# kscalelabs/gym-kmanip

Hardware: AMD Instinct MI355X
Metric: env steps/sec (whole node), KManipSoloArm @4096 envs, 1/2/4/8 MI355X (higher is better)
Workload: dtype f64

## Files before the change

gym_kmanip_amd/csrc/kmanip_api.hip:

```cpp
#include <hip/hip_runtime.h>

#include <cstdio>
#include <cstdlib>
#include <cmath>
#include <cstring>
#include <new>
#include <string>
#include <vector>

#include "kmanip_device.hpp"

#define KM_VERSION "kmanip-hip 0.33 (gfx950, f64)"

static thread_local std::string g_create_error;

struct KHandle_ {
  KModelDesc desc;
  KDeviceModel* dmodel = nullptr;
  KDeviceState st{};
  int device = 0;
  int num_envs = 0;
  std::string err;
  std::vector<hipEvent_t> ev;
  std::vector<char> ev_render;
  bool timing = false;
  int timing_every = 1;
  long timing_count = 0;
  double* rd_rec[2] = {nullptr, nullptr};
  int rd_sel = 0;
  int timed_steps = 0;
  double* qpos_snap[2] = {nullptr, nullptr};
  int render_src = -1;
  bool last_step_timed = false;
  int step_cam = -1, step_h = 0, step_w = 0;
  float* step_depth = nullptr;
// ... 1006 lines not shown
```

gym_kmanip_amd/csrc/kmanip_dyn_env.hpp:

```cpp
#pragma once
template <int NL, int G, int SOLVER>
__device__ __forceinline__ void step1_products(Ws<NL>& w, const LModel<NL>& lm, const KModelDesc* m, int sub,
                                               CReg<NL>& cr, real invm, Prof& pf) {
  real kin[15];
  fk_parallel<NL, G>(w, lm, sub, G == 16 ? kin : nullptr);
  pf.ph(0);
  real FN[6];
  const int split = G == 32 ? lm.split : 0;
  int bli = -1, bbase = 0;
  if constexpr (G == 32) {
    const int row = (threadIdx.x >> 4) & 1, c = threadIdx.x & 15;
    bbase = row ? split : 0;
    bli = (split && c < (row ? NL - split : split)) ? bbase + c : -1;
    if (split) {
      for (int e = sub; e < (int)(sizeof(w.Minv) / sizeof(real)); e += G) (&w.Minv[0][0])[e] = 0.0;
    }
  }
  if constexpr (G == 16) bias_bodies_rows<NL, NL>(w, lm, m, sub < NL ? sub : -1, 0, sub == NL, FN, kin);
  else if (split) {
    bias_bodies_rows<NL, KM_BLOCK_MAX>(w, lm, m, bli, bbase, false, FN);
    if (sub == NL) cube_bias<NL>(w, m);
  }
  else bias_bodies_parallel<NL, G>(w, lm, m, sub);
  pf.ph(1);
// ... 42 lines not shown
  real v = 0;
  if (sub < NV) {
    v = v0 + dt * a;
    w.qvel[sub] = v;
    w.warm[sub] = a;
    if (sub < NL + 3) w.qpos[sub] = qp + dt * v;
  }
  real ax[3] = {gbcast<G, NL + 3>(v), gbcast<G, NL + 4>(v), gbcast<G, NL + 5>(v)};
  if (sub == 0) {
    real ang = dt * normalize3_fast(ax), qr[4], qn[4];
    axis_angle2quat(qr, ax, ang);
    normalize4_fast(q);
    qmul(qn, q, qr);
    normalize4_fast(qn);
    w.qpos[NL + 3] = qn[0]; w.qpos[NL + 4] = qn[1]; w.qpos[NL + 5] = qn[2]; w.qpos[NL + 6] = qn[3];
  }
  GSYNC();
}

__device__ __forceinline__ real clip1(real x) { return fmin(fmax(x, -1.0), 1.0); }

template <int NL, int G>
__device__ __forceinline__ void write_obs(const Ws<NL>& w, const LModel<NL>& lm, const KModelDesc* m, int sub, double* obs_row) {
  for (int i = sub; i < NL; i += G) {
    obs_row[i] = clip1((w.qpos[i] - lm.range[i][0]) / (lm.range[i][1] - lm.range[i][0]));
    obs_row[NL + i] = clip1(w.qvel[i] / m->max_q_vel);
  }
  for (int c = sub; c < 7; c += G) {
    if (c < 3) obs_row[2 * NL + c] = clip1((w.qpos[NL + c] - m->cube_spawn_lo[c]) / (m->cube_spawn_hi[c] - m->cube_spawn_lo[c]));
    else obs_row[2 * NL + c] = w.qpos[NL + c];
  }
}

__device__ __forceinline__ real lerp_unfused(real lo, real hi, real u) {
#pragma clang fp contract(off)
  const real d = hi - lo;
  const real p = d * u;
  return lo + p;
}

#if KM_VAR_PAR
__device__ __forceinline__ real ep_inertia(const KModelDesc* m, real mass, int k) {
#pragma clang fp contract(off)
  return m->cube_inertia[k] * (mass / m->cube_mass);
}
__device__ __forceinline__ void ep_mass_consts(const KDeviceModel* dm, real mass, const real (&I)[3], int nv, real& cw1, real& mi) {
#pragma clang fp contract(off)
  cw1 = ((1.0 / I[0] + 1.0 / I[1]) + 1.0 / I[2]) / 3.0;
  mi = mass == dm->d.cube_mass ? dm->d.meaninertia : ((dm->trace_robot + 3.0 * mass) + ((I[0] + I[1]) + I[2])) / nv;
}
template <int NL>
__device__ __forceinline__ real ep_invm(const KModelDesc* m, const real (&p)[KM_EP_N], int sub) {
  if (sub < NL || sub >= Dim<NL>::NV) return 0;
// ... 95 lines not shown
#pragma unroll
  for (int k = 0; k < KL; k++) { const int i = sub + G * k; c[k] = st.ctrl[(size_t)(i < NL ? i : NL - 1) * NE + env]; }
#pragma unroll
  for (int k = 0; k < KQ; k++) { const int i = sub + G * k; if (i < NQ) { w.qpos[i] = q[k]; if (i < NL) w.qpos_ik[i] = q[k]; } }
#pragma unroll
  for (int k = 0; k < KV; k++) { const int i = sub + G * k; if (i < NV) { w.qvel[i] = v[k]; w.warm[i] = wm[k]; } }
#pragma unroll
  for (int k = 0; k < KL; k++) { const int i = sub + G * k; if (i < NL) w.ctrl[i] = (real)(float)c[k]; }
  if (sub == 0) { w.bad = 0; w.work = 0; }
}
template <int NL> struct LdsIO {
  Ws<NL>& w; const KDeviceState& st; int env;
  __device__ __forceinline__ real qpos(int i) const { return w.qpos[i]; }
  __device__ __forceinline__ void set_ctrl(int i, real v) { w.ctrl[i] = v; }
  __device__ __forceinline__ void set_qpos_ik(int i, real v) { w.qpos_ik[i] = v; }
  __device__ __forceinline__ void set_diag(int arm, int nfev, int status) {
    st.ik_nfev[(size_t)arm * st.num_envs + env] = nfev; st.ik_status[(size_t)arm * st.num_envs + env] = status;
  }
};
template <int NL, int G>
__device__ __forceinline__ void store_state(const Ws<NL>& w, const KDeviceState& st, int env, int sub) {
  constexpr int NV = Dim<NL>::NV, NQ = Dim<NL>::NQ;
  const int NE = st.num_envs;
  for (int i = sub; i < NQ; i += G) st.qpos[(size_t)i * NE + env] = w.qpos[i];
  for (int i = sub; i < NV; i += G) { st.qvel[(size_t)i * NE + env] = w.qvel[i]; st.warm[(size_t)i * NE + env] = w.warm[i]; }
  for (int i = sub; i < NL; i += G) st.ctrl[(size_t)i * NE + env] = w.ctrl[i];
}

template <int NL>
__device__ __forceinline__ void stage_model(LModel<NL>& lm, const KDeviceModel* dm) {
  static_assert(sizeof(LModel<NL>) % 16 == 0 && sizeof(LModel<NL>) <= KM_LMODEL_MAX, "the staged image is copied in 16-byte pieces");
  constexpr int N16 = (int)(sizeof(LModel<NL>) / 16);
  const uint4* src = reinterpret_cast<const uint4*>(dm->staged);
  uint4* dst = reinterpret_cast<uint4*>(&lm);
  uint4 v[(N16 + 63) / 64];
#pragma unroll
  for (int k = 0; k < (N16 + 63) / 64; k++) { const int i = threadIdx.x + 64 * k; v[k] = src[i < N16 ? i : N16 - 1]; }
#pragma unroll
  for (int k = 0; k < (N16 + 63) / 64; k++) { const int i = threadIdx.x + 64 * k; if (i < N16) dst[i] = v[k]; }
  __syncthreads();
}
template <int NL>
__device__ __forceinline__ void build_lmodel(LModel<NL>& lm, const KDeviceModel* dm) {
  const KModelDesc* m = &dm->d;
  for (int i = threadIdx.x; i < NL; i += 64) {
    lm.parent[i] = m->link_parent[i]; lm.jtype[i] = m->jnt_type[i]; lm.forcelimited[i] = m->forcelimited[i];
    lm.anc[i] = dm->x.anc_mask[i]; lm.desc[i] = dm->x.desc_mask[i];
    for (int k = 0; k < 4; k++) lm.jump[k][i] = dm->x.jump[k][i];
    if (i == 0) {
// ... 14 lines not shown
        lm.sphA[0][sp] = (cw + lw) + muc * muc * (cw + lw);
        lm.sphA[1][sp] = lw + mud * mud * lw;
      }
    }
    if (i < Dim<NL>::NSPH) {
      const int sp = i < m->nsphere ? i : 0;
      lm.sph_link[i] = m->sphere_link[sp]; lm.sph_rad[i] = m->sphere_radius[sp];
      for (int c = 0; c < 3; c++) { lm.sph_pos[i][c] = m->sphere_pos[sp][c]; lm.sph_seg[i][c] = m->sphere_seg[sp][c]; }
      if (i == 0) lm.nsph = m->nsphere < Dim<NL>::NSPH ? m->nsphere : Dim<NL>::NSPH;
    }
    lm.dofw[i] = m->dof_invweight0[i];
    lm.floss[i] = m->frictionloss[i]; lm.kp[i] = m->kp[i]; lm.mass[i] = m->mass[i]; lm.q_home[i] = m->q_home[i];
    for (int c = 0; c < 3; c++) { lm.pos[i][c] = m->link_pos[i][c]; lm.jaxis[i][c] = m->jnt_axis[i][c]; lm.com[i][c] = m->com[i][c]; lm.inertia[i][c] = m->inertia[i][c]; }
    for (int c = 0; c < 4; c++) lm.quat[i][c] = m->link_quat[i][c];
    { real qn[4] = {m->link_quat[i][0], m->link_quat[i][1], m->link_quat[i][2], m->link_quat[i][3]}, Rm[9]; normalize4(qn); quat2mat(Rm, qn); for (int c = 0; c < 9; c++) lm.R[i][c] = Rm[c]; }
    for (int c = 0; c < 2; c++) { lm.range[i][c] = m->jnt_range[i][c]; lm.ctrlrange[i][c] = m->ctrlrange[i][c]; lm.forcerange[i][c] = m->forcerange[i][c]; }
  }
  __syncthreads();
}

template <int NL, int G>
__device__ __forceinline__ real env_reward(Ws<NL>& w, const KModelDesc* m, int sub) {
  constexpr int NV = Dim<NL>::NV;
  real v2 = gsum<G>(sub < NV ? w.qvel[sub] * w.qvel[sub] : 0.0);
  GSYNC();
  real rew = -m->reward_vel_penalty * km_sqrt(v2);
  for (int arm = 1; arm >= 0; arm--) {
    if (!m->arm_present[arm] || !m->arm_has_grip[arm]) continue;
    const int l = m->arm_site_link[arm];
    real so[3] = {m->arm_site_pos[arm][0], m->arm_site_pos[arm][1], m->arm_site_pos[arm][2]}, sp[3];
    mat_vec3(sp, w.k.xmat[l], so);
    real df[3] = {w.qpos[NL] - (sp[0] + w.k.xpos[l][0]), w.qpos[NL + 1] - (sp[1] + w.k.xpos[l][1]), w.qpos[NL + 2] - (sp[2] + w.k.xpos[l][2])};
    rew += m->reward_grip_dist * (1.0 / (km_sqrt(dot3(df, df)) + m->epsilon));
  }
  if (m->touch_reward_enabled && (w.contact_mask & KM_CON_FINGERS_CUBE(NL))) {
    rew += m->reward_touch_cube;
    if (!w.touch_ct) rew += m->reward_lift_cube;
  }
  return rew;
}
```

gym_kmanip_amd/csrc/kmanip_dyn_newton.hpp:

```cpp
#pragma once

enum { KM_SUB_ALL = 0, KM_SUB_ARM = 1, KM_SUB_CUBE = 2 };
template <int NL, int S> struct SubSet {
  static constexpr int D0 = S == KM_SUB_CUBE ? NL : 0, D1 = S == KM_SUB_ARM ? NL : NL + 6;
  static constexpr int kind(int c) { return slot_kind<NL>(c); }
  static constexpr bool slot(int c) { return S == KM_SUB_ALL || (S == KM_SUB_ARM ? kind(c) == 2 : kind(c) == 0); }
  static constexpr int c0(int c) { const int k = kind(c); const int lo = k == 0 ? NL : 0; return lo > D0 ? lo : D0; }
  static constexpr int c1(int c) { const int k = kind(c); const int hi = k == 2 ? NL : NL + 6; return hi < D1 ? hi : D1; }
};

template <int G, int N, int D0, int D1>
__device__ __forceinline__ void chol_rows(real (&h)[N], real& invd, int sub, int& bad) {
  static_for<D0, D1>([&](auto kc) {
    constexpr int k = decltype(kc)::value;
    real dk = gbcast<G, k>(h[k]);
    if (!(dk > 0)) { bad = 1; dk = 1; }
    const real inv = rsqrt_nr(dk);
    const real lik = h[k] * inv;
    h[k] = lik;
    if (sub == k) invd = inv;
    const BSrc<G> lsrc = bsrc<G>(lik);
    fnmac_cols<G, k + 1, D1>(h, lsrc, lik);
    if constexpr (k + 2 >= D1 && k + 1 < D1) dpp_settle(h[k + 1]);
  });
// ... 330 lines not shown
template <int NL, int G, int S>
__device__ __forceinline__ void slot_grad(const CReg<NL>& cr, uint32_t act, const real (&F)[4], real& grad) {
  constexpr int NC = Dim<NL>::NC;
  static_assert(NC <= 16, "the slot lanes sit in the group's first DPP row");
  using SS = SubSet<NL, S>;
  const real F0 = row0<G>(F[0]), F1 = row0<G>(F[1]), F2 = row0<G>(F[2]), F3 = row0<G>(F[3]);
  static_for<0, NC>([&](auto cc) {
    constexpr int c = decltype(cc)::value;
    if constexpr (SS::slot(c)) {
      if ((act >> c) & 1u) {
        real g2 = 0;
        if constexpr (slot_kind<NL>(c) == 2) dppfma_acc3<c>(g2, F0, cr.jb[c][0], F1, cr.jb[c][1], F2, cr.jb[c][2]);
        else dppfma_acc4<c>(g2, F0, cr.jb[c][0], F1, cr.jb[c][1], F2, cr.jb[c][2], F3, cr.jb[c][3]);
        grad -= g2;
      }
    }
  });
}
template <int NL, int S> __device__ __forceinline__ bool slot_lane_in(int sub) {
  constexpr int NC = Dim<NL>::NC, NSS = Dim<NL>::NSS;
  return S == KM_SUB_ALL ? sub < NC : (S == KM_SUB_ARM ? (sub >= 4 + NSS && sub < NC) : sub < 4);
}

template <int NL, int G, bool CS>
__device__ __forceinline__ void newton_eval_sl(const Ws<NL>& w, int sub, const CReg<NL>& cr, real a, real a_s, real Mr, real& grad, int& qf,
                                               int& ql, real (&u)[4], real (&W)[7], real& c0, real& c1, real& cs) {
  constexpr int NV = Dim<NL>::NV;
  const uint32_t act = w.cact;
  const SlotC& sc = cr.sc;
  slot_project<NL, G, KM_SUB_ALL>(w, cr, act, sub, a, u);
#pragma unroll
  for (int k = 0; k < 4; k++) u[k] -= sc.A[k];
  real F[4];
  const real cslot = slot_eval<true>(sc, u, F, W);
  real csl = 0;
  if constexpr (CS) {
    real us[4], Fs[4], Ws_[7];
    slot_project<NL, G, KM_SUB_ALL>(w, cr, act, sub, a_s, us);
#pragma unroll
    for (int k = 0; k < 4; k++) us[k] -= sc.A[k];
    csl = slot_eval<false>(sc, us, Fs, Ws_);
  }
  grad = Mr;
  qf = 0; ql = 0;
  {
    real co = 0.5 * (a - a_s) * Mr;
    if (cr.fl > 0) { real f; co += row_eval(0, a - cr.areff, cr.Rf, cr.Df, cr.fl, f, qf); grad -= f; }
    if (cr.sg != 0) { real f; co += row_eval(1, cr.sg * a - cr.arefl, cr.Rl, cr.Dl, 0.0, f, ql); grad -= cr.sg * f; }
    c0 = sub < NL ? co : 0.0; c1 = (sub >= NL && sub < NV) ? co : 0.0;
    if constexpr (CS) {
      real f; int qd;
      if (cr.fl > 0) csl += row_eval(0, a_s - cr.areff, cr.Rf, cr.Df, cr.fl, f, qd);
      if (cr.sg != 0) csl += row_eval(1, cr.sg * a_s - cr.arefl, cr.Rl, cr.Dl, 0.0, f, qd);
    }
  }
  c1 += sub < 4 ? cslot : 0.0; c0 += sub < 4 ? 0.0 : cslot;
  slot_grad<NL, G, KM_SUB_ALL>(cr, act, F, grad);
  cs = csl;
}

// ... 294 lines not shown
    if constexpr (JOINT) { if (prob == KM_SUB_ALL) { pf.cnt(lone_it ? 44 : 45, 1); pf.it_end(lone_it ? 46 : 47); } }
#endif
    if (improvement < tol || gradient < tol || w.bad || iter + 1 >= maxit) {
      if (!(JOINT && prob == KM_SUB_ARM)) break;
      enter(KM_SUB_CUBE); cost = cost_b;
      if (small()) break;
      iter = -1;
    }
  }
}

template <int NL, int G>
__device__ __forceinline__ real solve_newton_sl(Ws<NL>& w, const LModel<NL>& lm, const KModelDesc* m, int sub, CReg<NL>& cr, real a_s,
                                                real invm, Prof& pf) {
  constexpr int NV = Dim<NL>::NV;
  const uint32_t act = w.cact;
  const real warm = sub < NV ? w.warm[sub] : 0.0;
  const real mdiag = (sub >= NL && sub < NV) ? 1.0 / invm : 0.0;
  real grad; int qf, ql;
  real u[4], W[7];
  real c0, c1, csl;
  real a = warm;
  real Mr = mass_mul<NL, G>(cr, sub, mdiag, warm - a_s);
  newton_eval_sl<NL, G, true>(w, sub, cr, a, a_s, Mr, grad, qf, ql, u, W, c0, c1, csl);
  real c3[3] = {csl, c0, c1};
  gsum_n<G, 3>(c3);
  const real cs = c3[0];
  real cost0 = c3[1], cost1 = c3[2];
  pf.ph(8);
  if (!(cost0 + cost1 < cs)) {
    a = a_s; Mr = 0;
    real dummy;
    newton_eval_sl<NL, G, false>(w, sub, cr, a, a_s, Mr, grad, qf, ql, u, W, c0, c1, dummy);
    real c2[2] = {c0, c1};
    gsum_n<G, 2>(c2);
    cost0 = c2[0]; cost1 = c2[1];
    pf.ph(38);
  }
  constexpr uint32_t FC_MASK = ((1u << Dim<NL>::NSS) - 1u) << 4;
  const bool coupled = (act & FC_MASK) != 0;
  if constexpr (G == 16) {
    int resume = KM_SUB_ARM, riter = 0;
    real rcost = cost0;
    if (__any(coupled)) {
      resume = 0;
      newton_loop_sl<NL, G, KM_SUB_ALL, true>(w, lm, m, sub, cr, mdiag, a_s, a, Mr, coupled ? cost0 + cost1 : cost0, grad, qf, ql, u, W, pf, !coupled, cost1,
                                              0, &resume, &rcost, &riter);
    }
    if (resume == KM_SUB_ARM) newton_loop_sl<NL, G, KM_SUB_ARM>(w, lm, m, sub, cr, mdiag, a_s, a, Mr, rcost, grad, qf, ql, u, W, pf, false, 0, riter);
    if (resume != 0) newton_loop_sl<NL, G, KM_SUB_CUBE>(w, lm, m, sub, cr, mdiag, a_s, a, Mr, resume == KM_SUB_ARM ? cost1 : rcost, grad, qf, ql, u, W, pf,
                                                        false, 0, resume == KM_SUB_ARM ? 0 : riter);
  } else {
    if (!coupled) newton_loop_sl<NL, G, KM_SUB_ARM>(w, lm, m, sub, cr, mdiag, a_s, a, Mr, cost0, grad, qf, ql, u, W, pf);
    if (coupled) newton_loop_sl<NL, G, KM_SUB_ALL>(w, lm, m, sub, cr, mdiag, a_s, a, Mr, cost0 + cost1, grad, qf, ql, u, W, pf);
    else newton_loop_sl<NL, G, KM_SUB_CUBE>(w, lm, m, sub, cr, mdiag, a_s, a, Mr, cost1, grad, qf, ql, u, W, pf);
  }
// ... 38 lines not shown
```

gym_kmanip_amd/csrc/kmanip_ik_coop.hip:

```cpp
#include "kmanip_ik_coop.hpp"

template <int N>
__global__ __launch_bounds__(64) void k_ik_coop_standalone(const KDeviceModel* __restrict__ dm, int arm, int n, int nq,
                                                           double* qpos, const double* goal_pos, const double* goal_quat,
                                                           double* q_out, int32_t* nfev_o, int32_t* status_o) {
  const KModelDesc* m = &dm->d;
  const int slot = threadIdx.x / GS, c = threadIdx.x % GS;
  const int e = blockIdx.x * PPW + slot;
  if (c >= GI || e >= n) return;
  double* qp = qpos + (size_t)e * nq;
  CoopCtx<N> P;
  Prof pf;
  P.m = m; P.ax = &dm->x; P.arm = arm; P.c = c; P.on = c < N; P.pf = &pf;
  coop_chain_setup<N>(P);
  const int q = m->arm_q_id[arm][P.on ? c : 0];
  const real x0 = P.on ? qp[q] : 0.0;
  P.q_prev = x0; P.q_home = m->q_home[q]; P.lb = m->jnt_range[q][0]; P.ub = m->jnt_range[q][1];
  P.qfix = (P.clen > N) ? qp[dm->x.chain_link[arm][P.clen - 1]] : 0.0;
  for (int k = 0; k < 3; k++) P.goal_pos[k] = goal_pos[3 * e + k];
  for (int k = 0; k < 4; k++) P.goal_quat[k] = goal_quat[4 * e + k];
  real xl;
  int nfev, status;
  const real qo = coop_ik_solve<N>(P, x0, xl, &nfev, &status);
  KM_GSYNC();
// ... 11 lines not shown
  else
    hipLaunchKernelGGL(k_ik_coop_standalone<6>, grid, dim3(64), 0, stream, dm, arm, n, nq, qpos, goal_pos, goal_quat, q_out, nfev, status);
}

template <int N>
__global__ __launch_bounds__(64) void k_ik_eval_coop(const KDeviceModel* __restrict__ dm, int arm, int n, int nq, const double* qpos,
                                                     const double* goal_pos, const double* goal_quat, double* res, double* jac) {
  const KModelDesc* m = &dm->d;
  const int slot = threadIdx.x / GS, c = threadIdx.x % GS;
  const int e = blockIdx.x * PPW + slot;
  if (c >= GI || e >= n) return;
  const double* qp = qpos + (size_t)e * nq;
  CoopCtx<N> P;
  Prof pf;
  P.m = m; P.ax = &dm->x; P.arm = arm; P.c = c; P.on = c < N; P.pf = &pf;
  coop_chain_setup<N>(P);
  const int q = m->arm_q_id[arm][P.on ? c : 0];
  const real x0 = P.on ? qp[q] : 0.0;
  P.q_prev = x0; P.q_home = m->q_home[q]; P.lb = m->jnt_range[q][0]; P.ub = m->jnt_range[q][1];
  P.qfix = (P.clen > N) ? qp[dm->x.chain_link[arm][P.clen - 1]] : 0.0;
  for (int k = 0; k < 3; k++) P.goal_pos[k] = goal_pos[3 * e + k];
  for (int k = 0; k < 4; k++) P.goal_quat[k] = goal_quat[4 * e + k];
  real ft[6], Jc[6];
  coop_eval<N, true>(P, x0, ft, Jc, nullptr, nullptr);
  constexpr int M = 6 + 2 * N;
  double* r = res + (size_t)e * M;
  double* J = jac + (size_t)e * M * N;
  if (c == 0) for (int k = 0; k < 6; k++) r[k] = ft[k];
  if (P.on) {
    r[6 + c] = m->ik_res_reg_prev * (x0 - P.q_prev);
    r[6 + N + c] = m->ik_res_reg_home * (x0 - P.q_home);
    for (int k = 0; k < M; k++) J[k * N + c] = 0;
    for (int k = 0; k < 6; k++) J[k * N + c] = Jc[k];
    J[(6 + c) * N + c] = m->ik_jac_reg;
    J[(6 + N + c) * N + c] = m->ik_jac_reg;
  }
}

void kmanip_launch_ik_eval_coop(const KDeviceModel* dm, const KModelDesc& hd, int arm, int n, const double* qpos,
                                const double* goal_pos, const double* goal_quat, double* res, double* jac, hipStream_t stream) {
  int nq = hd.nlink + 7;
  dim3 grid((n + PPW - 1) / PPW);
  if (hd.arm_nq[arm] == 7) hipLaunchKernelGGL(k_ik_eval_coop<7>, grid, dim3(64), 0, stream, dm, arm, n, nq, qpos, goal_pos, goal_quat, res, jac);
  else hipLaunchKernelGGL(k_ik_eval_coop<6>, grid, dim3(64), 0, stream, dm, arm, n, nq, qpos, goal_pos, goal_quat, res, jac);
}
```

gym_kmanip_amd/csrc/kmanip_ik_coop.hpp:

```cpp
#pragma once
#include "kmanip_device.hpp"

#define GI 8
#define GS 16
#define PPW (64 / GS)

__device__ __forceinline__ real gsum8(real v) {
#pragma clang fp contract(off)
  v += dpp_f64<0x141>(v);
  v += dpp_f64<0xB1>(v);
  v += dpp_f64<0x4E>(v);
  return v;
}
template <int N> __device__ __forceinline__ void gsum8_n(real (&v)[N]) {
#pragma clang fp contract(off)
  real t[N];
#pragma unroll
  for (int i = 0; i < N; i++) t[i] = dpp_f64<0x141>(v[i]);
#pragma unroll
  for (int i = 0; i < N; i++) v[i] += t[i];
#pragma unroll
  for (int i = 0; i < N; i++) t[i] = dpp_f64<0xB1>(v[i]);
#pragma unroll
  for (int i = 0; i < N; i++) v[i] += t[i];
// ... 24 lines not shown
  const KModelDesc* m;
  const KModelAux* ax;
  int arm, c;
  bool on;
  real goal_pos[3], goal_quat[4];
  real qfix;
  real q_prev, q_home, lb, ub;
  real cR[9], cp[3];
  int clen, cslide;
  Prof* pf;
};
template <int N>
__device__ __forceinline__ void coop_chain_setup(CoopCtx<N>& P) {
  P.clen = P.ax->chain_len[P.arm];
  const int k = P.c < P.clen ? P.c : 0;
  const int l = P.ax->chain_link[P.arm][k];
#pragma unroll
  for (int i = 0; i < 9; i++) P.cR[i] = P.ax->chain_R[P.arm][k][i];
  P.cp[0] = P.m->link_pos[l][0]; P.cp[1] = P.m->link_pos[l][1]; P.cp[2] = P.m->link_pos[l][2];
  P.cslide = P.m->jnt_type[l] == KM_JNT_SLIDE;
}
template <int S> __device__ __forceinline__ real shr8(real v) { return dpp_f64<0x110 + S>(v); }

template <int N, bool JAC>
__device__ __forceinline__ void coop_eval(const CoopCtx<N>& P, real x, real* ft, real* Jc, real* sp_out, real* smat_out) {
  const KModelDesc* m = P.m;
  const int arm = P.arm;
  const int clen = P.clen;
  real R[9], p[3];
  {
    const real q = P.on ? x : P.qfix;
    p[0] = P.cp[0]; p[1] = P.cp[1]; p[2] = P.cp[2];
    if (P.c >= clen) {
      R[0] = 1; R[1] = 0; R[2] = 0; R[3] = 0; R[4] = 1; R[5] = 0; R[6] = 0; R[7] = 0; R[8] = 1;
      p[0] = 0; p[1] = 0; p[2] = 0;
    } else if (P.cslide) {
#pragma unroll
      for (int i = 0; i < 9; i++) R[i] = P.cR[i];
      p[0] += R[2] * q; p[1] += R[5] * q; p[2] += R[8] * q;
    } else {
      real sn, cs;
      km_sincos(q, &sn, &cs);
#pragma unroll
      for (int i = 0; i < 3; i++) {
        R[3 * i] = cs * P.cR[3 * i] + sn * P.cR[3 * i + 1];
        R[3 * i + 1] = cs * P.cR[3 * i + 1] - sn * P.cR[3 * i];
        R[3 * i + 2] = P.cR[3 * i + 2];
      }
// ... 1 lines not shown
  }
  static_for<0, 3>([&](auto rc) {
    constexpr int S = 1 << decltype(rc)::value;
    real A[9], pa[3];
#pragma unroll
    for (int i = 0; i < 9; i++) A[i] = shr8<S>(R[i]);
    pa[0] = shr8<S>(p[0]); pa[1] = shr8<S>(p[1]); pa[2] = shr8<S>(p[2]);
    if (P.c >= S) {
      real t[3], Rn[9];
      mat_vec3(t, A, p);
      p[0] = t[0] + pa[0]; p[1] = t[1] + pa[1]; p[2] = t[2] + pa[2];
#pragma unroll
      for (int i = 0; i < 3; i++)
#pragma unroll
        for (int j = 0; j < 3; j++) Rn[3 * i + j] = A[3 * i] * R[j] + A[3 * i + 1] * R[3 + j] + A[3 * i + 2] * R[6 + j];
#pragma unroll
      for (int i = 0; i < 9; i++) R[i] = Rn[i];
    }
  });
  real mat[9], pos[3];
#pragma unroll
  for (int i = 0; i < 9; i++) mat[i] = bcast8<GI - 1>(R[i]);
  pos[0] = bcast8<GI - 1>(p[0]); pos[1] = bcast8<GI - 1>(p[1]); pos[2] = bcast8<GI - 1>(p[2]);
  const real anc[3] = {p[0], p[1], p[2]}, axw[3] = {R[2], R[5], R[8]};
  real sp[3], smat[9], cur[4], rq[3];
  real so[3] = {m->arm_site_pos[arm][0], m->arm_site_pos[arm][1], m->arm_site_pos[arm][2]};
  const double* Rs = P.ax->site_R[arm];
  mat_vec3(sp, mat, so);
  sp[0] += pos[0]; sp[1] += pos[1]; sp[2] += pos[2];
#pragma unroll
  for (int i = 0; i < 3; i++)
#pragma unroll
    for (int j = 0; j < 3; j++) smat[3 * i + j] = mat[3 * i] * Rs[j] + mat[3 * i + 1] * Rs[3 + j] + mat[3 * i + 2] * Rs[6 + j];
  mat2quat(cur, smat);
  real sn_h, ac_h;
  sub_quat_sc(rq, P.goal_quat, cur, sn_h, ac_h);
  if (sp_out) { sp_out[0] = sp[0]; sp_out[1] = sp[1]; sp_out[2] = sp[2]; }
  if (smat_out) {
#pragma unroll
    for (int i = 0; i < 9; i++) smat_out[i] = smat[i];
  }
  ft[0] = sp[0] - P.goal_pos[0]; ft[1] = sp[1] - P.goal_pos[1]; ft[2] = sp[2] - P.goal_pos[2];
  ft[3] = rq[0] * m->ik_res_rad; ft[4] = rq[1] * m->ik_res_rad; ft[5] = rq[2] * m->ik_res_rad;
  if (JAC) {
    real axs[3] = {rq[0], rq[1], rq[2]};
    real half = 0.5 * normalize3_fast(axs);
    real coef = 1.0 - (half < 6e-8 ? 1.0 : half * ac_h / sn_h);
    if (!P.on) { Jc[0] = 0; Jc[1] = 0; Jc[2] = 0; Jc[3] = 0; Jc[4] = 0; Jc[5] = 0; }
    else if (P.cslide) { Jc[0] = axw[0]; Jc[1] = axw[1]; Jc[2] = axw[2]; Jc[3] = 0; Jc[4] = 0; Jc[5] = 0; }
    else {
      real r[3] = {sp[0] - anc[0], sp[1] - anc[1], sp[2] - anc[2]}, jp[3];
      cross3(jp, axw, r);
      Jc[0] = jp[0]; Jc[1] = jp[1]; Jc[2] = jp[2];
      real uu[3], cx[3];
      matT_vec3(uu, smat, axw);
      cross3(cx, axs, uu);
      const real du = dot3(axs, uu);
#pragma unroll
      for (int i = 0; i < 3; i++) Jc[3 + i] = -m->ik_jac_rad * ((uu[i] + half * cx[i]) + coef * (axs[i] * du - uu[i]));
    }
  }
}

template <int N>
__device__ __forceinline__ real coop_cost(const CoopCtx<N>& P, real x, const real* ft) {
  real a = P.m->ik_res_reg_prev * (x - P.q_prev), b = P.m->ik_res_reg_home * (x - P.q_home);
  real loc = P.on ? a * a + b * b : 0.0;
  real s = gsum8(loc);
#pragma unroll
  for (int r = 0; r < 6; r++) s += ft[r] * ft[r];
  return 0.5 * s;
}
template <int N>
__device__ __forceinline__ real coop_grad(const CoopCtx<N>& P, real x, const real* ft, const real* Jc) {
  if (!P.on) return 0.0;
  real s = 0;
#pragma unroll
  for (int r = 0; r < 6; r++) s += Jc[r] * ft[r];
  return s + P.m->ik_jac_reg * (P.m->ik_res_reg_prev * (x - P.q_prev) + P.m->ik_res_reg_home * (x - P.q_home));
}

template <int N> struct TrFac { real h[N], ut[N], invd; };
template <int N>
__device__ __forceinline__ bool chol_coop(const real (&arow)[N], const real (&e)[N], real alpha, int c, TrFac<N>& F) {
// ... 77 lines not shown
template <int N>
__device__ __forceinline__ real ldl_fwd(const TrFacB<N>& F, real b) {
  static_for<0, N / 2>([&](auto kc) {
    constexpr int p = 2 * decltype(kc)::value, q = p + 1;
    if constexpr (q + 1 < N) { const real zb = b; dppfma_row2n<p, q>(b, zb, F.h[p], F.h[q]); }
  });
  return b;
}
template <int N>
__device__ __forceinline__ real ldl_mid(const TrFacB<N>& F, real z) {
  const real zp = dpp_f64<0xB1>(z);
  return __builtin_fma(F.dd, z, F.dx * zp);
}
template <int N>
__device__ __forceinline__ real ldl_bwd(const TrFacB<N>& F, real x) {
  if constexpr (N & 1) { const real xb = x; dppfma1<true, N - 1>(x, xb, F.ut[N - 1]); }
  static_for<0, N / 2>([&](auto kc) {
    constexpr int k = N / 2 - 1 - decltype(kc)::value, p = 2 * k, q = p + 1;
    if constexpr (k > 0) { const real xb = x; dppfma_row2n<p, q>(x, xb, F.ut[p], F.ut[q]); }
  });
  return x;
}

template <int N>
__device__ __forceinline__ void solve_tr_coop(const real (&arow)[N], const real (&e)[N], int c, real g_h, real Delta, real& alpha, real& p) {
  const real ng = -g_h;
#ifdef KM_IK_CHOLESKY
  TrFac<N> F;
  auto factor = [&](real al) { return chol_coop<N>(arow, e, al, c, F); };
  auto solve = [&](real rhs) { return tr_bwd<N>(F, tr_fwd<N>(F, rhs)); };
  auto ainv_norm2 = [&](real v) { const real q = tr_fwd<N>(F, v); return gsum8(q * q); };
#else
  TrFacB<N> F;
  auto factor = [&](real al) { return ldl_coop<N>(arow, e, al, c, F); };
  auto solve = [&](real rhs) { return ldl_bwd<N>(F, ldl_mid<N>(F, ldl_fwd<N>(F, rhs))); };
  auto ainv_norm2 = [&](real v) { const real z = ldl_fwd<N>(F, v); return gsum8(z * ldl_mid<N>(F, z)); };
#endif
  const bool full_rank = factor(0.0);
  real pn = 0;
  if (full_rank) {
    p = solve(ng);
    pn = km_sqrt(gsum8(p * p));
    if (pn <= Delta) { alpha = 0.0; return; }
  }
  const real iDelta = frcp(Delta);
  real alpha_upper = km_sqrt(gsum8(g_h * g_h)) * iDelta, alpha_lower = 0.0;
  if (full_rank) {
    const real phi = pn - Delta, phip = -ainv_norm2(p) * frcp(pn);
    alpha_lower = -phi * frcp(phip);
  }
  if (!full_rank && alpha == 0) alpha = fmax(0.001 * alpha_upper, sqrt(alpha_lower * alpha_upper));
  for (int it = 0; it < 10; it++) {
    if (alpha < alpha_lower || alpha > alpha_upper) alpha = fmax(0.001 * alpha_upper, sqrt(alpha_lower * alpha_upper));
    factor(alpha);
    p = solve(ng);
    pn = km_sqrt(gsum8(p * p));
    const real phi = pn - Delta, phip = -ainv_norm2(p) * frcp(pn);
    if (phi < 0) alpha_upper = alpha;
    const real ratio = phi * frcp(phip);
    alpha_lower = fmax(alpha_lower, alpha - ratio);
    alpha -= (phi + Delta) * ratio * iDelta;
    if (fabs(phi) < 0.01 * Delta) break;
  }
  factor(alpha);
  p = solve(ng);
  p *= Delta * rsqrt_nr(gsum8(p * p));
}

__device__ __forceinline__ void min_quad_1d_c(real a, real b, real lo, real hi, real c, real& t_out, real& y_out) {
  real tb = lo, yb = lo * (a * lo + b) + c;
  real y1 = hi * (a * hi + b) + c;
// ... 80 lines not shown
  agh *= ag_stride;
  if (p_value < r_value && p_value < ag_value) { step_h = pht; return -p_value; }
  if (r_value < p_value && r_value < ag_value) { step_h = rh; return -r_value; }
  step_h = agh;
  return -ag_value;
}

__device__ __forceinline__ real lane_strictly_feasible(real x, real lb, real ub, real rstep) {
  real xn = x;
  if (rstep == 0) {
    if (x <= lb) xn = nextafter(lb, ub);
    if (x >= ub) xn = nextafter(ub, lb);
  } else {
    real ld = x - lb, ud = ub - x;
    real lt = rstep * fmax(1.0, fabs(lb)), ut = rstep * fmax(1.0, fabs(ub));
    if (ld <= fmin(ud, lt)) xn = lb + lt;
    if (ud <= fmin(ld, ut)) xn = ub - ut;
  }
  if (xn < lb || xn > ub) xn = 0.5 * (lb + ub);
  return xn;
}

template <int N>
__device__ int coop_trf(const CoopCtx<N>& P, real& x, real& x_last, int* nfev_out) {
  const real ftol = 1e-8, xtol = 1e-8, gtol = 1e-8;
  const int max_nfev = P.m->ik_max_nfev > 0 ? P.m->ik_max_nfev : 100 * N;
  const real jreg2 = 2 * P.m->ik_jac_reg * P.m->ik_jac_reg;
  real ft[6], Jc[6], ft_new[6], Jn[6], e[N];
#pragma unroll
  for (int j = 0; j < N; j++) e[j] = P.c == j ? 1.0 : 0.0;
  coop_eval<N, true>(P, x, ft, Jc, nullptr, nullptr);
  P.pf->ph(33);
  int nfev = 1;
  real cost = coop_cost<N>(P, x, ft);
  real g = coop_grad<N>(P, x, ft, Jc);
  real v = 1;
  if (g < 0) v = P.ub - x;
  if (g > 0) v = x - P.lb;
  real Delta = km_sqrt(gsum8(P.on ? x * x / v : 0.0));
  if (Delta == 0) Delta = 1.0;
  real alpha = 0.0, cost_new = cost;
  int status = -1;
  x_last = x;
  for (;;) {
    real dv = 0;
    v = 1;
    if (g < 0) { v = P.ub - x; dv = -1; }
    if (g > 0) { v = x - P.lb; dv = 1; }
    const real g_norm = gmax8(P.on ? fabs(g * v) : 0.0);
    if (g_norm < gtol) status = 1;
    if (status != -1 || nfev == max_nfev) break;
    const real d = km_sqrt(v), diag_h = g * dv, g_h = d * g;
    real arow[N];
    static_for<0, N>([&](auto jc) {
      constexpr int j = decltype(jc)::value;
      real s = 0;
      dppfma_acc3<j>(s, Jc[0], Jc[0], Jc[1], Jc[1], Jc[2], Jc[2]);
      dppfma_acc3<j>(s, Jc[3], Jc[3], Jc[4], Jc[4], Jc[5], Jc[5]);
      s = __builtin_fma(e[j], jreg2, s);
      s *= d * bcast8<j>(d);
      arow[j] = P.on ? __builtin_fma(e[j], diag_h, s) : 0.0;
    });
    P.pf->ph(34);
    const real theta = fmax(0.995, 1 - g_norm);
    real actual = -1, x_new = x;
    while (actual <= 0 && nfev < max_nfev) {
      real ph = 0;
      solve_tr_coop<N>(arow, e, P.c, g_h, Delta, alpha, ph);
      P.pf->ph(35);
      real step_h;
      const real predicted = coop_select_step<N>(P, arow, x, d, ph, g_h, Delta, theta, step_h);
      if (!P.on) step_h = 0;
      P.pf->ph(36);
      const real step = d * step_h;
      x_new = P.on ? lane_strictly_feasible(x + step, P.lb, P.ub, 0.0) : x;
      coop_eval<N, true>(P, x_new, ft_new, Jn, nullptr, nullptr);
      P.pf->ph(33);
      x_last = x_new;
      nfev++;
      real n3[3] = {step_h * step_h, step * step, P.on ? x * x : 0.0};
      gsum8_n<3>(n3);
      const real shn = km_sqrt(n3[0]);
      bool fin = true;
#pragma unroll
      for (int r = 0; r < 6; r++) fin = fin && isfinite(ft_new[r]);
      if (!fin) { Delta = 0.25 * shn; continue; }
      cost_new = coop_cost<N>(P, x_new, ft_new);
      actual = cost - cost_new;
      real ratio, Delta_new = Delta;
      if (predicted > 0) ratio = actual * frcp(predicted);
      else if (predicted == 0 && actual == 0) ratio = 1;
      else ratio = 0;
      if (ratio < 0.25) Delta_new = 0.25 * shn;
      else if (ratio > 0.75 && shn > 0.95 * Delta) Delta_new = Delta * 2.0;
      const real sn = km_sqrt(n3[1]), xn = km_sqrt(n3[2]);
      const bool ft_ok = (actual < ftol * cost) && (ratio > 0.25);
      const bool xt_ok = sn < xtol * (xtol + xn);
      if (ft_ok && xt_ok) status = 4; else if (ft_ok) status = 2; else if (xt_ok) status = 3;
      if (status != -1) break;
      alpha *= Delta * frcp(Delta_new);
      Delta = Delta_new;
      P.pf->ph(37);
    }
    if (actual > 0) {
      x = x_new;
      cost = cost_new;
#pragma unroll
      for (int r = 0; r < 6; r++) { ft[r] = ft_new[r]; Jc[r] = Jn[r]; }
      g = coop_grad<N>(P, x, ft, Jc);
    }
  }
  if (status == -1) status = 0;
  *nfev_out = nfev;
  return status;
}

template <int N>
__device__ __forceinline__ real coop_ik_solve(const CoopCtx<N>& P, real x0, real& x_last, int* nfev, int* status) {
  real x = x0;
  x_last = x0;
  *nfev = 0; *status = -2;
  if (gall8(!P.on || (x >= P.lb && x <= P.ub))) {
    if (P.on) x = lane_strictly_feasible(x, P.lb, P.ub, 1e-10);
    *status = coop_trf<N>(P, x, x_last, nfev);
  }
  return fmin(fmax(x, P.lb), P.ub);
}

__device__ __forceinline__ real f32r_c(real x) { return (real)(float)x; }

template <int N, class IO>
__device__ __forceinline__ void coop_before_step(const KDeviceModel* dm, int arm, int c, const float* a, IO& io, Prof* pf) {
  const KModelDesc* m = &dm->d;
  const int grip_key[2] = {KM_ACT_GRIP_R, KM_ACT_GRIP_L};
  const int pos_key[2] = {KM_ACT_EER_POS, KM_ACT_EEL_POS};
  const int orn_key[2] = {KM_ACT_EER_ORN, KM_ACT_EEL_ORN};
  const int qp_key[2] = {KM_ACT_QPOS_R, KM_ACT_QPOS_L};
  const int cg = m->act_col[grip_key[arm]];
  if (cg >= 0 && c == 0) {
    int g0 = m->arm_grip_id[arm][0], g1 = m->arm_grip_id[arm][1];
    float g = a[cg] * (float)m->ee_s_delta;
    g = (float)((double)g + io.qpos(g0));
    g = fminf(fmaxf(g, (float)m->ee_s_min), (float)m->ee_s_max);
    io.set_ctrl(g0, (double)g);
    io.set_ctrl(g1, (double)g);
  }
  CoopCtx<N> P;
  P.m = m; P.ax = &dm->x; P.arm = arm; P.c = c; P.on = c < N; P.pf = pf;
  coop_chain_setup<N>(P);
  const int q = m->arm_q_id[arm][P.on ? c : 0];
  const real x0 = P.on ? io.qpos(q) : 0.0;
  P.q_prev = x0; P.q_home = m->q_home[q]; P.lb = m->jnt_range[q][0]; P.ub = m->jnt_range[q][1];
  P.qfix = (P.clen > N) ? io.qpos(dm->x.chain_link[arm][P.clen - 1]) : 0.0;
  const int cp = m->act_col[pos_key[arm]], co = m->act_col[orn_key[arm]], cq = m->act_col[qp_key[arm]];
  if (cp >= 0) {
    P.goal_pos[0] = 0; P.goal_pos[1] = 0; P.goal_pos[2] = 0;
    P.goal_quat[0] = 1; P.goal_quat[1] = 0; P.goal_quat[2] = 0; P.goal_quat[3] = 0;
    real ft0[6], sp[3], smat[9];
    coop_eval<N, false>(P, x0, ft0, nullptr, sp, smat);
    real e0 = km_atan2(smat[7], smat[8]);
    real e1 = km_atan2(-smat[6], km_sqrt(smat[7] * smat[7] + smat[8] * smat[8]));
    real e2 = km_atan2(smat[3], smat[0]);
    e0 += (double)a[co] * m->ee_orn_delta[0];
    e1 += (double)a[co + 1] * m->ee_orn_delta[1];
    e2 += (double)a[co + 2] * m->ee_orn_delta[2];
    real s0, c0, s1, c1, s2, c2;
    km_sincos(e0 * 0.5, &s0, &c0); km_sincos(e1 * 0.5, &s1, &c1); km_sincos(e2 * 0.5, &s2, &c2);
    real qx[4] = {c0, s0, 0, 0}, qy[4] = {c1, 0, s1, 0};
    real qz[4] = {c2, 0, 0, s2}, t4[4];
    qmul(t4, qy, qx);
    qmul(P.goal_quat, qz, t4);
    P.goal_pos[0] = (double)a[cp] * m->ee_pos_delta[0] + sp[0];
    P.goal_pos[1] = (double)a[cp + 1] * m->ee_pos_delta[1] + sp[1];
    P.goal_pos[2] = (double)a[cp + 2] * m->ee_pos_delta[2] + sp[2];
    real xl;
    int nfev, status;
    const real qo = coop_ik_solve<N>(P, x0, xl, &nfev, &status);
    if (P.on) { io.set_ctrl(q, f32r_c(qo)); io.set_qpos_ik(q, xl); }
    if (c == 0) io.set_diag(arm, nfev, status);
  } else {
    if (c == 0) io.set_diag(arm, 0, -3);
    if (cq >= 0 && P.on)
      io.set_ctrl(q, f32r_c(x0 + (double)(a[cq + c] * (float)m->q_pos_delta)));
  }
}
```

Measured before the change: 7.781 million.

## Reuse IK kinematics, hoist trust-region factorization, and batch LDS loads in env kernels

Splits the IK forward evaluation into kinematics and residual parts so the initial kinematics computed for goal construction is reused by the first TRF evaluation. It caches the zero-damping factorization, Newton step, gradient norm and phi-derivative across inner trust-region retries instead of recomputing them each time. The Newton line search reuses an already projected slot vector instead of projecting again. Observation, reward and state-store routines now load all LDS values into registers up front, using clamped indices and asm pins, before issuing the global stores. The cost is more register pressure and more complex control flow.

```diff
diff --git a/gym_kmanip_amd/csrc/kmanip_api.hip b/gym_kmanip_amd/csrc/kmanip_api.hip
--- a/gym_kmanip_amd/csrc/kmanip_api.hip
+++ b/gym_kmanip_amd/csrc/kmanip_api.hip
@@ -10,7 +10,7 @@
 
 #include "kmanip_device.hpp"
 
-#define KM_VERSION "kmanip-hip 0.33 (gfx950, f64)"
+#define KM_VERSION "kmanip-hip 0.34 (gfx950, f64)"
 
 static thread_local std::string g_create_error;
 
diff --git a/gym_kmanip_amd/csrc/kmanip_dyn_env.hpp b/gym_kmanip_amd/csrc/kmanip_dyn_env.hpp
--- a/gym_kmanip_amd/csrc/kmanip_dyn_env.hpp
+++ b/gym_kmanip_amd/csrc/kmanip_dyn_env.hpp
@@ -88,13 +88,20 @@
 
 template <int NL, int G>
 __device__ __forceinline__ void write_obs(const Ws<NL>& w, const LModel<NL>& lm, const KModelDesc* m, int sub, double* obs_row) {
-  for (int i = sub; i < NL; i += G) {
-    obs_row[i] = clip1((w.qpos[i] - lm.range[i][0]) / (lm.range[i][1] - lm.range[i][0]));
-    obs_row[NL + i] = clip1(w.qvel[i] / m->max_q_vel);
-  }
-  for (int c = sub; c < 7; c += G) {
-    if (c < 3) obs_row[2 * NL + c] = clip1((w.qpos[NL + c] - m->cube_spawn_lo[c]) / (m->cube_spawn_hi[c] - m->cube_spawn_lo[c]));
-    else obs_row[2 * NL + c] = w.qpos[NL + c];
+  static_assert(NL <= G && 7 <= G, "one arm component and one cube component per lane");
+  int sv = sub;
+  asm volatile("" : "+v"(sv));
+  const int si = sv < NL ? sv : NL - 1, sc = sv < 7 ? sv : 6, s3 = sv < 3 ? sv : 2;
+  real qp = w.qpos[si], r0 = lm.range[si][0], r1 = lm.range[si][1], qv = w.qvel[si], qc = w.qpos[NL + sc];
+  real lo = m->cube_spawn_lo[s3], hi = m->cube_spawn_hi[s3];
+  km_pin(qp, r0, r1, qv, qc); km_pin(lo, hi);
+  if (sub < NL) {
+    obs_row[sub] = clip1((qp - r0) / (r1 - r0));
+    obs_row[NL + sub] = clip1(qv / m->max_q_vel);
+  }
+  if (sub < 7) {
+    if (sub < 3) obs_row[2 * NL + sub] = clip1((qc - lo) / (hi - lo));
+    else obs_row[2 * NL + sub] = qc;
   }
 }
 
@@ -236,9 +243,20 @@
 __device__ __forceinline__ void store_state(const Ws<NL>& w, const KDeviceState& st, int env, int sub) {
   constexpr int NV = Dim<NL>::NV, NQ = Dim<NL>::NQ;
   const int NE = st.num_envs;
-  for (int i = sub; i < NQ; i += G) st.qpos[(size_t)i * NE + env] = w.qpos[i];
-  for (int i = sub; i < NV; i += G) { st.qvel[(size_t)i * NE + env] = w.qvel[i]; st.warm[(size_t)i * NE + env] = w.warm[i]; }
-  for (int i = sub; i < NL; i += G) st.ctrl[(size_t)i * NE + env] = w.ctrl[i];
+  constexpr int KQ = (NQ + G - 1) / G, KV = (NV + G - 1) / G, KL = (NL + G - 1) / G;
+  real q[KQ], v[KV], wm[KV], c[KL];
+#pragma unroll
+  for (int k = 0; k < KQ; k++) { const int i = sub + G * k; q[k] = w.qpos[i < NQ ? i : NQ - 1]; }
+#pragma unroll
+  for (int k = 0; k < KV; k++) { const int i = sub + G * k, ic = i < NV ? i : NV - 1; v[k] = w.qvel[ic]; wm[k] = w.warm[ic]; }
+#pragma unroll
+  for (int k = 0; k < KL; k++) { const int i = sub + G * k; c[k] = w.ctrl[i < NL ? i : NL - 1]; }
+#pragma unroll
+  for (int k = 0; k < KQ; k++) { const int i = sub + G * k; if (i < NQ) st.qpos[(size_t)i * NE + env] = q[k]; }
+#pragma unroll
+  for (int k = 0; k < KV; k++) { const int i = sub + G * k; if (i < NV) { st.qvel[(size_t)i * NE + env] = v[k]; st.warm[(size_t)i * NE + env] = wm[k]; } }
+#pragma unroll
+  for (int k = 0; k < KL; k++) { const int i = sub + G * k; if (i < NL) st.ctrl[(size_t)i * NE + env] = c[k]; }
 }
 
 template <int NL>
@@ -299,20 +317,31 @@
 template <int NL, int G>
 __device__ __forceinline__ real env_reward(Ws<NL>& w, const KModelDesc* m, int sub) {
   constexpr int NV = Dim<NL>::NV;
-  real v2 = gsum<G>(sub < NV ? w.qvel[sub] * w.qvel[sub] : 0.0);
-  GSYNC();
+  int sv = sub;
+  asm volatile("" : "+v"(sv));
+  const real qv = w.qvel[sv < NV ? sv : NV - 1];
+  real v2 = gsum<G>(sub < NV ? qv * qv : 0.0);
+  GSYNC();
+  real cp[3] = {w.qpos[NL], w.qpos[NL + 1], w.qpos[NL + 2]};
+  uint32_t cmask = w.contact_mask;
+  int tct = w.touch_ct;
   real rew = -m->reward_vel_penalty * km_sqrt(v2);
   for (int arm = 1; arm >= 0; arm--) {
     if (!m->arm_present[arm] || !m->arm_has_grip[arm]) continue;
     const int l = m->arm_site_link[arm];
+    real xm[9], xp[3] = {w.k.xpos[l][0], w.k.xpos[l][1], w.k.xpos[l][2]};
+#pragma unroll
+    for (int k = 0; k < 9; k++) xm[k] = w.k.xmat[l][k];
+    km_pin(xp, xm); km_pin(cp);
     real so[3] = {m->arm_site_pos[arm][0], m->arm_site_pos[arm][1], m->arm_site_pos[arm][2]}, sp[3];
-    mat_vec3(sp, w.k.xmat[l], so);
-    real df[3] = {w.qpos[NL] - (sp[0] + w.k.xpos[l][0]), w.qpos[NL + 1] - (sp[1] + w.k.xpos[l][1]), w.qpos[NL + 2] - (sp[2] + w.k.xpos[l][2])};
+    mat_vec3(sp, xm, so);
+    real df[3] = {cp[0] - (sp[0] + xp[0]), cp[1] - (sp[1] + xp[1]), cp[2] - (sp[2] + xp[2])};
     rew += m->reward_grip_dist * (1.0 / (km_sqrt(dot3(df, df)) + m->epsilon));
   }
-  if (m->touch_reward_enabled && (w.contact_mask & KM_CON_FINGERS_CUBE(NL))) {
+  asm volatile("" : "+v"(cmask), "+v"(tct));
+  if (m->touch_reward_enabled && (cmask & KM_CON_FINGERS_CUBE(NL))) {
     rew += m->reward_touch_cube;
-    if (!w.touch_ct) rew += m->reward_lift_cube;
+    if (!tct) rew += m->reward_lift_cube;
   }
   return rew;
 }
diff --git a/gym_kmanip_amd/csrc/kmanip_dyn_newton.hpp b/gym_kmanip_amd/csrc/kmanip_dyn_newton.hpp
--- a/gym_kmanip_amd/csrc/kmanip_dyn_newton.hpp
+++ b/gym_kmanip_amd/csrc/kmanip_dyn_newton.hpp
@@ -376,20 +376,22 @@
   return S == KM_SUB_ALL ? sub < NC : (S == KM_SUB_ARM ? (sub >= 4 + NSS && sub < NC) : sub < 4);
 }
 
-template <int NL, int G, bool CS>
+template <int NL, int G, bool CS, bool PROJ = true>
 __device__ __forceinline__ void newton_eval_sl(const Ws<NL>& w, int sub, const CReg<NL>& cr, real a, real a_s, real Mr, real& grad, int& qf,
-                                               int& ql, real (&u)[4], real (&W)[7], real& c0, real& c1, real& cs) {
+                                               int& ql, real (&u)[4], real (&W)[7], real& c0, real& c1, real& cs, real (&us)[4]) {
   constexpr int NV = Dim<NL>::NV;
   const uint32_t act = w.cact;
   const SlotC& sc = cr.sc;
-  slot_project<NL, G, KM_SUB_ALL>(w, cr, act, sub, a, u);
-#pragma unroll
-  for (int k = 0; k < 4; k++) u[k] -= sc.A[k];
+  if constexpr (PROJ) {
+    slot_project<NL, G, KM_SUB_ALL>(w, cr, act, sub, a, u);
+#pragma unroll
+    for (int k = 0; k < 4; k++) u[k] -= sc.A[k];
+  }
   real F[4];
   const real cslot = slot_eval<true>(sc, u, F, W);
   real csl = 0;
   if constexpr (CS) {
-    real us[4], Fs[4], Ws_[7];
+    real Fs[4], Ws_[7];
     slot_project<NL, G, KM_SUB_ALL>(w, cr, act, sub, a_s, us);
 #pragma unroll
     for (int k = 0; k < 4; k++) us[k] -= sc.A[k];
@@ -730,7 +732,8 @@
   real c0, c1, csl;
   real a = warm;
   real Mr = mass_mul<NL, G>(cr, sub, mdiag, warm - a_s);
-  newton_eval_sl<NL, G, true>(w, sub, cr, a, a_s, Mr, grad, qf, ql, u, W, c0, c1, csl);
+  real us[4];
+  newton_eval_sl<NL, G, true>(w, sub, cr, a, a_s, Mr, grad, qf, ql, u, W, c0, c1, csl, us);
   real c3[3] = {csl, c0, c1};
   gsum_n<G, 3>(c3);
   const real cs = c3[0];
@@ -739,7 +742,9 @@
   if (!(cost0 + cost1 < cs)) {
     a = a_s; Mr = 0;
     real dummy;
-    newton_eval_sl<NL, G, false>(w, sub, cr, a, a_s, Mr, grad, qf, ql, u, W, c0, c1, dummy);
+#pragma unroll
+    for (int k = 0; k < 4; k++) u[k] = us[k];
+    newton_eval_sl<NL, G, false, false>(w, sub, cr, a, a_s, Mr, grad, qf, ql, u, W, c0, c1, dummy, us);
     real c2[2] = {c0, c1};
     gsum_n<G, 2>(c2);
     cost0 = c2[0]; cost1 = c2[1];
diff --git a/gym_kmanip_amd/csrc/kmanip_ik_coop.hip b/gym_kmanip_amd/csrc/kmanip_ik_coop.hip
--- a/gym_kmanip_amd/csrc/kmanip_ik_coop.hip
+++ b/gym_kmanip_amd/csrc/kmanip_ik_coop.hip
@@ -57,7 +57,7 @@
   for (int k = 0; k < 3; k++) P.goal_pos[k] = goal_pos[3 * e + k];
   for (int k = 0; k < 4; k++) P.goal_quat[k] = goal_quat[4 * e + k];
   real ft[6], Jc[6];
-  coop_eval<N, true>(P, x0, ft, Jc, nullptr, nullptr);
+  coop_eval<N, true>(P, x0, ft, Jc);
   constexpr int M = 6 + 2 * N;
   double* r = res + (size_t)e * M;
   double* J = jac + (size_t)e * M * N;
diff --git a/gym_kmanip_amd/csrc/kmanip_ik_coop.hpp b/gym_kmanip_amd/csrc/kmanip_ik_coop.hpp
--- a/gym_kmanip_amd/csrc/kmanip_ik_coop.hpp
+++ b/gym_kmanip_amd/csrc/kmanip_ik_coop.hpp
@@ -70,8 +70,9 @@
 }
 template <int S> __device__ __forceinline__ real shr8(real v) { return dpp_f64<0x110 + S>(v); }
 
-template <int N, bool JAC>
-__device__ __forceinline__ void coop_eval(const CoopCtx<N>& P, real x, real* ft, real* Jc, real* sp_out, real* smat_out) {
+struct CoopKin { real sp[3], smat[9], anc[3], axw[3]; };
+template <int N>
+__device__ __forceinline__ void coop_kin(const CoopCtx<N>& P, real x, CoopKin& K) {
   const KModelDesc* m = P.m;
   const int arm = P.arm;
   const int clen = P.clen;
@@ -119,8 +120,8 @@
 #pragma unroll
   for (int i = 0; i < 9; i++) mat[i] = bcast8<GI - 1>(R[i]);
   pos[0] = bcast8<GI - 1>(p[0]); pos[1] = bcast8<GI - 1>(p[1]); pos[2] = bcast8<GI - 1>(p[2]);
-  const real anc[3] = {p[0], p[1], p[2]}, axw[3] = {R[2], R[5], R[8]};
-  real sp[3], smat[9], cur[4], rq[3];
+  K.anc[0] = p[0]; K.anc[1] = p[1]; K.anc[2] = p[2]; K.axw[0] = R[2]; K.axw[1] = R[5]; K.axw[2] = R[8];
+  real sp[3], smat[9];
   real so[3] = {m->arm_site_pos[arm][0], m->arm_site_pos[arm][1], m->arm_site_pos[arm][2]};
   const double* Rs = P.ax->site_R[arm];
   mat_vec3(sp, mat, so);
@@ -129,14 +130,20 @@
   for (int i = 0; i < 3; i++)
 #pragma unroll
     for (int j = 0; j < 3; j++) smat[3 * i + j] = mat[3 * i] * Rs[j] + mat[3 * i + 1] * Rs[3 + j] + mat[3 * i + 2] * Rs[6 + j];
+  K.sp[0] = sp[0]; K.sp[1] = sp[1]; K.sp[2] = sp[2];
+#pragma unroll
+  for (int i = 0; i < 9; i++) K.smat[i] = smat[i];
+}
+template <int N, bool JAC>
+__device__ __forceinline__ void coop_resid(const CoopCtx<N>& P, const CoopKin& K, real* ft, real* Jc) {
+  const KModelDesc* m = P.m;
+  const real anc[3] = {K.anc[0], K.anc[1], K.anc[2]}, axw[3] = {K.axw[0], K.axw[1], K.axw[2]}, sp[3] = {K.sp[0], K.sp[1], K.sp[2]};
+  real smat[9], cur[4], rq[3];
+#pragma unroll
+  for (int i = 0; i < 9; i++) smat[i] = K.smat[i];
   mat2quat(cur, smat);
   real sn_h, ac_h;
   sub_quat_sc(rq, P.goal_quat, cur, sn_h, ac_h);
-  if (sp_out) { sp_out[0] = sp[0]; sp_out[1] = sp[1]; sp_out[2] = sp[2]; }
-  if (smat_out) {
-#pragma unroll
-    for (int i = 0; i < 9; i++) smat_out[i] = smat[i];
-  }
   ft[0] = sp[0] - P.goal_pos[0]; ft[1] = sp[1] - P.goal_pos[1]; ft[2] = sp[2] - P.goal_pos[2];
   ft[3] = rq[0] * m->ik_res_rad; ft[4] = rq[1] * m->ik_res_rad; ft[5] = rq[2] * m->ik_res_rad;
   if (JAC) {
@@ -157,6 +164,12 @@
       for (int i = 0; i < 3; i++) Jc[3 + i] = -m->ik_jac_rad * ((uu[i] + half * cx[i]) + coef * (axs[i] * du - uu[i]));
     }
   }
+}
+template <int N, bool JAC>
+__device__ __forceinline__ void coop_eval(const CoopCtx<N>& P, real x, real* ft, real* Jc) {
+  CoopKin K;
+  coop_kin<N>(P, x, K);
+  coop_resid<N, JAC>(P, K, ft, Jc);
 }
 
 template <int N>
@@ -280,8 +293,10 @@
   return x;
 }
 
-template <int N>
-__device__ __forceinline__ void solve_tr_coop(const real (&arow)[N], const real (&e)[N], int c, real g_h, real Delta, real& alpha, real& p) {
+struct TrHoist { bool have = false, full_rank = false, have_gn = false, have_q0 = false; real p0 = 0, pn0 = 0, gn = 0, q0 = 0; };
+template <int N>
+__device__ __forceinline__ void solve_tr_coop(const real (&arow)[N], const real (&e)[N], int c, real g_h, real Delta, real& alpha, real& p,
+                                              TrHoist& H) {
   const real ng = -g_h;
 #ifdef KM_IK_CHOLESKY
   TrFac<N> F;
@@ -294,17 +309,33 @@
   auto solve = [&](real rhs) { return ldl_bwd<N>(F, ldl_mid<N>(F, ldl_fwd<N>(F, rhs))); };
   auto ainv_norm2 = [&](real v) { const real z = ldl_fwd<N>(F, v); return gsum8(z * ldl_mid<N>(F, z)); };
 #endif
-  const bool full_rank = factor(0.0);
+  bool at0 = false;
+  if (!H.have) {
+    H.full_rank = factor(0.0);
+    at0 = true;
+    if (H.full_rank) {
+      H.p0 = solve(ng);
+      H.pn0 = km_sqrt(gsum8(H.p0 * H.p0));
+    }
+    H.have = true;
+  }
+  const bool full_rank = H.full_rank;
   real pn = 0;
   if (full_rank) {
-    p = solve(ng);
-    pn = km_sqrt(gsum8(p * p));
+    p = H.p0;
+    pn = H.pn0;
     if (pn <= Delta) { alpha = 0.0; return; }
   }
   const real iDelta = frcp(Delta);
-  real alpha_upper = km_sqrt(gsum8(g_h * g_h)) * iDelta, alpha_lower = 0.0;
+  if (!H.have_gn) { H.gn = km_sqrt(gsum8(g_h * g_h)); H.have_gn = true; }
+  real alpha_upper = H.gn * iDelta, alpha_lower = 0.0;
   if (full_rank) {
-    const real phi = pn - Delta, phip = -ainv_norm2(p) * frcp(pn);
+    if (!H.have_q0) {
+      if (!at0) factor(0.0);
+      H.q0 = ainv_norm2(p);
+      H.have_q0 = true;
+    }
+    const real phi = pn - Delta, phip = -H.q0 * frcp(pn);
     alpha_lower = -phi * frcp(phip);
   }
   if (!full_rank && alpha == 0) alpha = fmax(0.001 * alpha_upper, sqrt(alpha_lower * alpha_upper));
@@ -431,14 +462,19 @@
 }
 
 template <int N>
-__device__ int coop_trf(const CoopCtx<N>& P, real& x, real& x_last, int* nfev_out) {
+__device__ int coop_trf(const CoopCtx<N>& P, real& x, real& x_last, int* nfev_out, const CoopKin* K0, real x0) {
   const real ftol = 1e-8, xtol = 1e-8, gtol = 1e-8;
   const int max_nfev = P.m->ik_max_nfev > 0 ? P.m->ik_max_nfev : 100 * N;
   const real jreg2 = 2 * P.m->ik_jac_reg * P.m->ik_jac_reg;
   real ft[6], Jc[6], ft_new[6], Jn[6], e[N];
 #pragma unroll
   for (int j = 0; j < N; j++) e[j] = P.c == j ? 1.0 : 0.0;
-  coop_eval<N, true>(P, x, ft, Jc, nullptr, nullptr);
+  {
+    CoopKin K;
+    const bool same = K0 != nullptr && gall8(!P.on || x == x0);
+    if (same) K = *K0; else coop_kin<N>(P, x, K);
+    coop_resid<N, true>(P, K, ft, Jc);
+  }
   P.pf->ph(33);
   int nfev = 1;
   real cost = coop_cost<N>(P, x, ft);
@@ -473,9 +509,10 @@
     P.pf->ph(34);
     const real theta = fmax(0.995, 1 - g_norm);
     real actual = -1, x_new = x;
+    TrHoist hoist;
     while (actual <= 0 && nfev < max_nfev) {
       real ph = 0;
-      solve_tr_coop<N>(arow, e, P.c, g_h, Delta, alpha, ph);
+      solve_tr_coop<N>(arow, e, P.c, g_h, Delta, alpha, ph, hoist);
       P.pf->ph(35);
       real step_h;
       const real predicted = coop_select_step<N>(P, arow, x, d, ph, g_h, Delta, theta, step_h);
@@ -483,7 +520,7 @@
       P.pf->ph(36);
       const real step = d * step_h;
       x_new = P.on ? lane_strictly_feasible(x + step, P.lb, P.ub, 0.0) : x;
-      coop_eval<N, true>(P, x_new, ft_new, Jn, nullptr, nullptr);
+      coop_eval<N, true>(P, x_new, ft_new, Jn);
       P.pf->ph(33);
       x_last = x_new;
       nfev++;
@@ -525,13 +562,13 @@
 }
 
 template <int N>
-__device__ __forceinline__ real coop_ik_solve(const CoopCtx<N>& P, real x0, real& x_last, int* nfev, int* status) {
+__device__ __forceinline__ real coop_ik_solve(const CoopCtx<N>& P, real x0, real& x_last, int* nfev, int* status, const CoopKin* K0 = nullptr) {
   real x = x0;
   x_last = x0;
   *nfev = 0; *status = -2;
   if (gall8(!P.on || (x >= P.lb && x <= P.ub))) {
     if (P.on) x = lane_strictly_feasible(x, P.lb, P.ub, 1e-10);
-    *status = coop_trf<N>(P, x, x_last, nfev);
+    *status = coop_trf<N>(P, x, x_last, nfev, K0, x0);
   }
   return fmin(fmax(x, P.lb), P.ub);
 }
@@ -563,10 +600,10 @@
   P.qfix = (P.clen > N) ? io.qpos(dm->x.chain_link[arm][P.clen - 1]) : 0.0;
   const int cp = m->act_col[pos_key[arm]], co = m->act_col[orn_key[arm]], cq = m->act_col[qp_key[arm]];
   if (cp >= 0) {
-    P.goal_pos[0] = 0; P.goal_pos[1] = 0; P.goal_pos[2] = 0;
-    P.goal_quat[0] = 1; P.goal_quat[1] = 0; P.goal_quat[2] = 0; P.goal_quat[3] = 0;
-    real ft0[6], sp[3], smat[9];
-    coop_eval<N, false>(P, x0, ft0, nullptr, sp, smat);
+    CoopKin K0;
+    coop_kin<N>(P, x0, K0);
+    const real (&sp)[3] = K0.sp;
+    const real (&smat)[9] = K0.smat;
     real e0 = km_atan2(smat[7], smat[8]);
     real e1 = km_atan2(-smat[6], km_sqrt(smat[7] * smat[7] + smat[8] * smat[8]));
     real e2 = km_atan2(smat[3], smat[0]);
@@ -584,7 +621,7 @@
     P.goal_pos[2] = (double)a[cp + 2] * m->ee_pos_delta[2] + sp[2];
     real xl;
     int nfev, status;
-    const real qo = coop_ik_solve<N>(P, x0, xl, &nfev, &status);
+    const real qo = coop_ik_solve<N>(P, x0, xl, &nfev, &status, &K0);
     if (P.on) { io.set_ctrl(q, f32r_c(qo)); io.set_qpos_ik(q, xl); }
     if (c == 0) io.set_diag(arm, nfev, status);
   } else {
```

Measured after the change: 7.755 million. About the same (-0.3%).
